# genometools/vstree

Hardware: AMD Instinct MI355X
Metric: queries/sec (100 bp queries, vmatch -mum -l 20 semantics, 3 Gbp ESA index resident in HBM) (higher is better)
Workload: dtype u8; 1 GPU; 3 Gbp synthetic DNA index, 10 M x 100 bp queries per GPU, -mum -l 20; index_bp=3000000000, queries_per_gpu=10000000, query_len=100, minlen=20, prefixlength=13, index_bytes_hbm=115012207262, reads_in_hbm=two bits per symbol, 32 bytes per read (vsa_pack_reads), parallelism=index replicated, queries sharded x1

## Files before the change

vstree_amd/csrc/api.hip:

```cpp
#include "vsa_internal.hpp"
#include <atomic>
#include <thread>
#include <time.h>
#include <algorithm>

static thread_local char g_errbuf[VSA_ERRBUF_SIZE] = "";

extern "C" char *vsa_errbuf()
{
  return g_errbuf;
}

extern "C" const char *vsa_messagespace(void)
{
  return g_errbuf;
}

int vsa_set_device(int device)
{
  VSA_HIP(hipSetDevice(device));
  return 0;
}

extern "C" int vsa_device_count(void)
// ... 382 lines not shown
  int rc = vsa_index_alloc(src->n, src->pl, src->numofchars, src->nllv,
                           src->bwt != nullptr, device, &ix, false);
  auto fail = [&](int code) {
    vsa_index_close(ix);
    return code;
  };
  if (rc != 0)
  {
    return fail(rc);
  }
  if (ix->isize != src->isize)
  {
    (void) hipFree(ix->suf);
    (void) hipFree(ix->llv);
    (void) hipFree(ix->bck);
    ix->suf = ix->llv = ix->bck = nullptr;
    ix->isize = src->isize;
    if (vsa_hip_malloc(&ix->suf, (src->n + 1) * ix->isize) != hipSuccess ||
        vsa_hip_malloc(&ix->llv, 2 * src->nllv * ix->isize + 16) != hipSuccess ||
        vsa_hip_malloc(&ix->bck, 2 * ix->numofcodes * ix->isize) != hipSuccess)
    {
      VSA_ERROR("vsa_index_clone: out of device memory");
      return fail(-100);
    }
  }
  const uint64_t n = src->n;
  struct Piece
  {
    void **dst;
    const void *from;
    uint64_t bytes;
    bool allocate;
  };
  const uint64_t ncodes = src->D > 0 ? 1ull << (2 * src->D) : 0,
                 nblocks = (n >> 6) + 1, nwaves = (nblocks + 63) / 64;
  Piece pieces[] = {
      {(void **) &ix->tis_alloc, src->tis_alloc,
       VSA_TIS_FRONTPAD + n + VSA_TIS_BACKPAD, false},
      {&ix->suf, src->suf, (n + 1) * src->isize, false},
      {(void **) &ix->lcp, src->lcp, n + 1 + 32, false},
      {&ix->llv, src->llv, 2 * src->nllv * src->isize, false},
      {&ix->bck, src->bck, 2 * src->numofcodes * src->isize, false},
      {(void **) &ix->bwt, src->bwt, n + 1 + 32, false},
      {(void **) &ix->esa8, src->esa8, (n + 1) * 8 + 64, true},
      {(void **) &ix->bck2, src->bck2, 2 * ncodes * 4 + 16, true},
      {(void **) &ix->slot16, src->slot16,
       (uint64_t) src->slotwords * ncodes * 8 + 32, true},
      {(void **) &ix->tis2, src->tis2, nblocks * 16 + 64, true},
      {(void **) &ix->spec64, src->spec64, nwaves * 8 + 64, true}};
  for (const Piece &p : pieces)
  {
    if (p.from == nullptr || p.bytes == 0)
    {
      continue;
    }
    if (p.allocate)
    {
      if (vsa_hip_malloc(p.dst, p.bytes) != hipSuccess)
      {
        VSA_ERROR("vsa_index_clone: out of device memory");
        return fail(-100);
      }
      ix->device_bytes += p.bytes;
    }
    const hipError_t e =
        hipMemcpyPeerAsync(*p.dst, device, p.from, src->device, p.bytes,
                           ix->stream);
    if (e != hipSuccess)
    {
      VSA_ERROR("vsa_index_clone: copy from device %d to device %d: %s",
                src->device, device, hipGetErrorString(e));
      return fail(-100);
    }
  }
  if (hipStreamSynchronize(ix->stream) != hipSuccess)
  {
    VSA_ERROR("vsa_index_clone: copy failed");
    return fail(-100);
  }
  ix->device_bytes = src->device_bytes;
  ix->D = src->D;
  ix->tune = src->tune;
  ix->walkshift = src->walkshift;
  ix->qspeedup = src->qspeedup;
  ix->slotwords = src->slotwords;
  ix->firstspecial = src->firstspecial;
  ix->querysepposition = src->querysepposition;
  ix->hasindexedqueries = src->hasindexedqueries;
  ix->lcpquirk = src->lcpquirk;
  *clone = ix;
  return 0;
}

extern "C" void vsa_index_close(vsa_index *ix)
{
  if (ix == nullptr)
  {
    return;
  }
  (void) hipSetDevice(ix->device);
  (void) hipFree(ix->tis_alloc);
  (void) hipFree(ix->suf);
  (void) hipFree(ix->lcp);
  (void) hipFree(ix->llv);
  (void) hipFree(ix->bck);
  (void) hipFree(ix->bwt);
  (void) hipFree(ix->esa8);
  (void) hipFree(ix->bck2);
  (void) hipFree(ix->slot16);
  (void) hipFree(ix->tis2);
  (void) hipFree(ix->spec64);
  (void) hipFree(ix->isa32);
  (void) hipFree(ix->repbits);
  if (ix->stream != nullptr)
  {
    vsa_dev_forget_stream(ix->stream);
    (void) hipStreamDestroy(ix->stream);
  }
  delete ix;
}

extern "C" int vsa_index_from_tables(const vsa_tables *t, int device,
                                     vsa_index **index)
{
  if (t == nullptr || index == nullptr)
  {
    VSA_ERROR("vsa_index_from_tables: NULL argument");
    return -1;
  }
  *index = nullptr;
  if (t->integersize != 32 && t->integersize != 64)
  {
    VSA_ERROR("integersize=%u: only 32 and 64 bit indexes are supported",
              t->integersize);
    return -2;
  }
  if ((t->tis == nullptr && t->bck != nullptr) || t->suf == nullptr ||
      t->lcp == nullptr || (t->largelcpvalues > 0 && t->llv == nullptr))
  {
    VSA_ERROR("tables tis, suf, lcp (and llv) are required");
    return -3;
  }
  if (t->numofchars == 0 || t->numofchars > 253 ||
      (t->bck != nullptr && t->prefixlength == 0))
  {
    VSA_ERROR("prefixlength=%u numofchars=%u: not a usable bucket table",
              t->prefixlength, t->numofchars);
    return -4;
  }
  vsa_index *ix = nullptr;
  int rc = vsa_index_alloc(t->totallength,
                           t->bck != nullptr ? t->prefixlength : 0,
                           t->numofchars, t->largelcpvalues,
                           t->bwt != nullptr, device, &ix);
  if (rc != 0)
  {
    vsa_index_close(ix);
    return rc;
  }
  ix->querysepposition = t->querysepposition;
  ix->hasindexedqueries = t->hasindexedqueries;
  const uint64_t n = ix->n;
  hipStream_t s = ix->stream;
  auto fail = [&](int code) {
    vsa_index_close(ix);
    return code;
// ... 980 lines not shown
```

vstree_amd/csrc/esa_search.hip:

```cpp
#include "search_host.hpp"
#include <rocprim/rocprim.hpp>
#include <type_traits>

#include "search_complete.inc"
#include "search_query.inc"
#include "mum_workplan.inc"
#include "mem_workplan.inc"
#include "mum_filter.inc"
#include "candidate_sort.inc"
#include <atomic>


namespace
{


enum class Form
{
  Ref,
  Deep,
  Staged,
  Rows,
  Windows
};
// ... 660 lines not shown
  VSA_HIP(plan_summary(st));
  st.fromplan = true;
  st.plansearches = nq;
  return 0;
}

int dump_planfile(QueryRun &st, const char *pf)
{
  const uint64_t k = std::min<uint64_t>(st.queries->nq, 65536);
  std::vector<uint32_t> hc(k), hp(k * VSA_PLAN_RANGES);
  VSA_HIP(hipMemcpyAsync(hc.data(), st.wcount.p, k * 4,
                         hipMemcpyDeviceToHost, st.stream));
  VSA_HIP(hipMemcpyAsync(hp.data(), st.wplan.p, k * sizeof(PlanRanges),
                         hipMemcpyDeviceToHost, st.stream));
  VSA_HIP(hipStreamSynchronize(st.stream));
  if (FILE *f = fopen(pf, "wb"))
  {
    for (uint64_t q = 0; q < k; q++)
    {
      (void) fwrite(&hc[q], 4, 1, f);
      (void) fwrite(&hp[q * VSA_PLAN_RANGES], 4, VSA_PLAN_RANGES, f);
    }
    fclose(f);
  }
  return 0;
}

template <typename IDX>
int mum_plan(QueryRun &st, const DevIndex<IDX> &ix)
{
  const uint64_t nq = st.queries->nq;
  if (alloc_first(st) || st.wlist.alloc(nq * 4))
  {
    return -100;
  }
  VSA_HIP(hipMemsetAsync(st.wcount.as<uint32_t>() + nq, 0, 4, st.stream));
  const uint64_t nb = blocksfor(nq), nbr = vsa_grid_blocks(nb);
  DevBuf bcount;
  if (bcount.alloc((nbr + 1) * 8) || st.wboffset.alloc((nbr + 1) * 8))
  {
    return -100;
  }
  VSA_HIP(hipMemsetAsync(bcount.as<uint64_t>() + nb, 0, 8, st.stream));
  if (first_pass(st, ix, st.form, bcount.as<uint64_t>()))
  {
    return -100;
  }
  VSA_HIP(rocprim_run(st.wtemp, [&](void *p, size_t &tb) {
    return rocprim::exclusive_scan(p, tb, bcount.as<uint64_t>(),
                                   st.wboffset.as<uint64_t>(), (uint64_t) 0,
                                   (size_t) (nb + 1), rocprim::plus<uint64_t>(),
                                   st.stream);
  }));
  k_wanted_fill<<<vsa_grid(nb), VSA_BLOCK, 0, st.stream>>>(
      st.wcount.as<uint32_t>(), nq, 0u, st.wboffset.as<uint64_t>(),
      st.wlist.as<uint32_t>());
  VSA_HIP(hipGetLastError());
  st.nlistword = st.wboffset.as<uint64_t>() + nb;
  PlanEmit em = PlanEmit();
  if (st.form != Form::Ref && plan_emit(st, VSA_PLAN_ROUNDS - 1, &em))
  {
    return -100;
  }
  withform(st.form, [&](auto deep, auto, auto rows, auto) {
    k_mum_plan<IDX, deep, deep, rows><<<gridfor(nq), VSA_BLOCK, 0, st.stream>>>(
        ix, st.qs, st.wlist.as<uint32_t>(), st.nlistword, st.searchlength,
        st.wfirste.as<uint32_t>(), st.wcount.as<uint32_t>(),
        st.wplan.as<PlanRanges>(), em);
  });
  if (st.planemit)
  {
    VSA_HIP(plan_summary(st));
  }
  VSA_HIP(hipGetLastError());
  const char *pf = getenv("VSA_DEBUG_PLANFILE");
  if (pf != nullptr && dump_planfile(st, pf))
  {
    return -100;
  }
  st.fromplan = true;
  return 0;
}

template <typename IDX>
void launch_search(QueryRun &st, const DevIndex<IDX> &ix,
                   uint64_t nplanblocks)
{
  withform(st.form, [&](auto deep, auto, auto rows, auto) {
    auto planned = [&](auto mum) {
      k_query_search_planned<IDX, 256, deep, rows, mum>
          <<<vsa_grid(nplanblocks), 256, 0, st.stream>>>(
              ix, st.qs, st.dbase, st.perquery, st.wplan.as<PlanRanges>(),
              st.wcount.as<uint32_t>(), st.searchlength,
              st.rawout.as<vsa_match>(), st.rawkeys.as<uint64_t>(),
              st.shardcap, VSA_CURSOR_SHARDS - 1,
              st.cursor.as<unsigned long long>(), st.rec.packbits,
              st.rec.valbits, st.blocksum.as<PlannedWork>(),
              st.index->walkshift);
    };
    auto unplanned = [&](auto mum) {
      k_query_search<IDX, mum, deep, 256>
          <<<vsa_grid((st.nitems + 255) / 256), 256, 0, st.stream>>>(
              ix, st.qs, st.dbase, st.perquery, st.nitems, st.searchlength,
              st.rawout.as<vsa_match>(), st.rawkeys.as<uint64_t>(),
              st.shardcap, VSA_CURSOR_SHARDS - 1,
              st.cursor.as<unsigned long long>(), st.rec.packbits,
              st.rec.valbits);
    };
    if (st.fromplan && st.domum)
    {
      planned(std::true_type());
    } else if (st.fromplan)
    {
      if constexpr (deep && !rows)
      {
        planned(std::false_type());
      }
    } else if (st.nitems > 0 && st.domum)
    {
      unplanned(std::true_type());
    } else if (st.nitems > 0)
    {
      unplanned(std::false_type());
    }
  });
}

template <typename IDX>
int search(QueryRun &st, const DevIndex<IDX> &ix)
{
  const uint32_t nshards = VSA_CURSOR_SHARDS;
  const uint64_t perblock = 256 * (st.domum ? VSA_WALK_READS : 1);
  const uint64_t nplanblocks = (st.queries->nq + perblock - 1) / perblock;
  size_t rbytes = 0;
  if (st.fromplan)
  {
    if (st.blocksum.alloc((vsa_grid_blocks(nplanblocks) + 1) *
                          sizeof(PlannedWork)))
    {
      return -100;
    }
    VSA_HIP(rocprim::reduce(nullptr, rbytes, st.blocksum.as<PlannedWork>(),
                            (PlannedWork *) nullptr, PlannedWork{0, 0},
                            (size_t) nplanblocks, PlannedWorkPlus(),
                            st.stream));
    if (st.rtemp.alloc(rbytes))
    {
      return -100;
    }
  }
  if (st.cursor.alloc((size_t) nshards * VSA_CURSOR_STRIDE * 8) ||
      st.doff.alloc(nshards * 8) || st.summary.alloc(6 * 8))
  {
    return -100;
  }
  st.shardcap =
      std::max<uint64_t>((st.queries->nq * 2 / nshards) * 5 / 4 + 64, 256);
  uint64_t maxshard = 0;
  for (int attempt = 0; attempt < 2; attempt++)
  {
    if (st.rawout.alloc(nshards * st.shardcap * st.rec.recsize) ||
        st.rawkeys.alloc(nshards * st.shardcap * 8))
    {
      return -100;
    }
    VSA_HIP(hipMemsetAsync(st.cursor.p, 0,
                           (size_t) nshards * VSA_CURSOR_STRIDE * 8,
                           st.stream));
    st.tsearch.start();
    launch_search(st, ix, nplanblocks);
    st.tsearch.stop();
    VSA_HIP(hipGetLastError());
    if (st.fromplan)
    {
      VSA_HIP(rocprim::reduce(
          st.rtemp.p, rbytes, st.blocksum.as<PlannedWork>(),
          reinterpret_cast<PlannedWork *>(st.summary.as<uint64_t>() + 4),
          PlannedWork{0, 0}, (size_t) nplanblocks, PlannedWorkPlus(),
          st.stream));
    }
    const uint64_t *sm = st.summary.as<uint64_t>();
    VSA_HIP(shard_summary(st.cursor.as<unsigned long long>(), nshards,
                          st.doff.as<uint64_t>(), st.summary.as<uint64_t>(),
                          st.stream));
    const Fetch f[8] = {{sm, 8}, {sm + 1, 8}, {sm + 2, 8}, {sm + 3, 8},
                        {sm + 4, 8}, {st.planemit ? st.psummary.p : sm, 8},
                        {st.nlistword != nullptr ? st.nlistword : sm, 8},
                        {sm + 5, 8}};
    uint64_t got[8];
    if (fetchwords(st.stream, f, 8, got))
    {
      return -100;
    }
    if (st.nlistword != nullptr)
    {
      st.nfirst = got[6] >> 32;
      st.plansearches = 2 * (got[6] & 0xFFFFFFFFull);
    }
    st.nplan = st.planemit ? got[5] : 0;
    st.needed = got[0];
    maxshard = got[1];
    st.plannedlocates = st.fromplan ? got[4] : 0;
    st.plannedwork = st.fromplan ? got[7] : 0;
    st.searchms += st.tsearch.ms();
    if (maxshard <= st.shardcap)
    {
      return 0;
    }
    st.shardcap = maxshard;
  }
  VSA_ERROR("match buffer overflow: %llu > %llu",
            (unsigned long long) maxshard, (unsigned long long) st.shardcap);
  return -5;
}

int compact(QueryRun &st)
{
  const uint64_t total = st.needed + st.nplan + st.nfirst;
  if (total == 0)
  {
    return 0;
  }
  if (st.out.alloc(total * st.rec.recsize) || st.keys.alloc(total * 8) ||
      (st.nplan > 0 &&
       compact_into(st.rec, st.prawout, st.prawkeys, st.pcap, st.pcursor,
                    st.pdoff, st.out, st.keys, st.needed, st.stream)) ||
      (st.needed > 0 &&
       compact_into(st.rec, st.rawout, st.rawkeys, st.shardcap, st.cursor,
                    st.doff, st.out, st.keys, 0, st.stream)))
  {
    return -100;
  }
  if (st.nfirst > 0)
  {
    k_append_first<<<gridfor(st.queries->nq), VSA_BLOCK, 0, st.stream>>>(
        st.wfmlen.as<uint32_t>(), st.wfmdb.as<uint64_t>(),
        st.wboffset.as<uint64_t>(), st.queries->nq, st.perquery, st.dbase,
        st.qs.seqoffset, st.needed + st.nplan, st.out.as<vsa_match>(),
        st.keys.as<uint64_t>(), st.rec.packbits, st.rec.valbits);
    VSA_HIP(hipGetLastError());
  }
  st.needed = total;
  return 0;
}

#define VSA_CS_MINPAIRS (1u << 14)

std::atomic<uint64_t> g_cs_runs{0}, g_cs_overflows{0}, g_cs_longruns{0},
    g_cs_shift{0}, g_cs_buckets{0};

bool feedsbuckets(const QueryRun &st)
{
  const uint64_t total = st.needed + st.nplan + st.nfirst;
  const uint32_t tune = st.index->tune;
  if (!(st.domum && !st.domumcand && st.rec.packed && (tune & 4u) == 0 &&
        total > 0 && (total >= VSA_CS_MINPAIRS || (tune & 8u) != 0) &&
        cs_geometry(st.index->n, total, st.rec.lenbits, st.rec.dbbits)
                .nbuckets <= VSA_CS_MAXBUCKETS))
  {
    return false;
  }
  if ((tune & 8u) == 0 && st.index->cs_skip > 0)
  {
    st.index->cs_skip--;
    return false;
  }
  return true;
}

template <typename VAL>
int mumfilter_buckets(QueryRun &st, DevBuf &mums, MumCounts *c)
{
  const RecordForm &rec = st.rec;
  const uint64_t total = st.needed + st.nplan + st.nfirst;
  CsSources src = CsSources();
  if (st.needed > 0)
  {
    src.reg[0] = {st.rawout.p, st.rawkeys.as<uint64_t>(),
                  st.cursor.as<unsigned long long>(), st.shardcap, st.needed};
  }
  if (st.nplan > 0)
  {
    src.reg[1] = {st.prawout.p, st.prawkeys.as<uint64_t>(),
                  st.pcursor.as<unsigned long long>(), st.pcap, st.nplan};
  }
  if (st.nfirst > 0)
  {
    src.first = {st.wfmlen.as<uint32_t>(), st.wfmdb.as<uint64_t>(),
                 st.queries->nq, st.qs.seqoffset, rec.packbits, rec.valbits};
  }
  CsGeometry g;
  if (mums.alloc(total * sizeof(vsa_match)))
// ... 548 lines not shown
```

vstree_amd/csrc/index_derive.hip:

```cpp
#include "search_host.hpp"
#include <rocprim/rocprim.hpp>


template <typename IDX>
__global__ void __launch_bounds__(VSA_BLOCK)
k_make_esa8(const uint8_t *__restrict__ tis, const IDX *__restrict__ suf,
            const uint8_t *__restrict__ lcp, uint64_t count, uint32_t D,
            uint64_t *__restrict__ esa8)
{
  const uint64_t j = vsa_bid() * VSA_BLOCK + threadIdx.x;
  if (j >= count)
  {
    return;
  }
  const uint64_t s = suf[j];
  const uint8_t *t = tis + s + D;
  uint64_t key = 0, flag = 0;
#pragma unroll
  for (uint32_t k = 0; k < VSA_KEYSYMS; k++)
  {
    const uint8_t a = t[k];
    if (VSA_ISSPECIAL(a))
    {
      flag = VSA_KEYFLAG;
// ... 21 lines not shown
#pragma unroll
    for (int k = 0; k < 4; k++)
    {
      const vsa_u128 v = vsa_load16(p + 16 * k);
      const uint64_t notdna = 0xFCFCFCFCFCFCFCFCull;
      const uint64_t s0 = v.lo & notdna, s1 = v.hi & notdna;
      if (firstbad == ~0ull && (s0 | s1) != 0)
      {
        firstbad = 64 * b + 16 * k +
                   (s0 != 0 ? ((uint64_t) __builtin_ctzll(s0) >> 3)
                            : 8 + ((uint64_t) __builtin_ctzll(s1) >> 3));
      }
      const uint64_t packed = vsa_pack16(v.lo, v.hi);
      out[k >> 1] |= packed << (32 * (1 - (k & 1)));
    }
    out[0] = __builtin_bswap64(out[0]);
    out[1] = __builtin_bswap64(out[1]);
    reinterpret_cast<uint64_t *>(tis2)[2 * b] = out[0];
    reinterpret_cast<uint64_t *>(tis2)[2 * b + 1] = out[1];
    special = firstbad != ~0ull || 64 * b + 64 > n;
    if (firstbad != ~0ull)
    {
      atomicMin(firstspecial, (unsigned long long) firstbad);
    }
  }
  const uint64_t mask = __ballot(special);
  if ((threadIdx.x & 63) == 0 && b < nblocks)
  {
    reinterpret_cast<uint64_t *>(spec64)[b >> 6] = mask;
  }
}

template <int W, typename IDX>
__global__ void __launch_bounds__(VSA_BLOCK)
k_make_slots(const IDX *__restrict__ bck2, const uint64_t *__restrict__ esa8,
             uint64_t ncodes, uint64_t *__restrict__ slot,
             unsigned int *__restrict__ toobig)
{
  for (uint64_t c = vsa_bid() * VSA_BLOCK + threadIdx.x;
       c < ncodes; c += vsa_nblocks() * VSA_BLOCK)
  {
    const IDX left = bck2[2 * c], mid = bck2[2 * c + 1];
    if constexpr (sizeof(IDX) == 4)
    {
      slot[W * c] = (uint64_t) left | ((uint64_t) mid << 32);
    } else
    {
      const uint64_t cnt = mid > left ? mid - left : 0;
      if (cnt >> (64 - VSA_WIDE_LEFTBITS) != 0)
      {
        *toobig = 1;
      }
      slot[W * c] = left | (cnt << VSA_WIDE_LEFTBITS);
    }
#pragma unroll
    for (int k = 0; k + 1 < W; k++)
    {
      slot[W * c + 1 + k] = (mid > left + k) ? esa8[left + k] : 0;
    }
  }
}

int vsa_index_make_esa8(vsa_index *ix)
{
  const char *off = getenv("VSA_NO_ESA8");
  {
    const char *tn = getenv("VSA_TUNE"), *wc = getenv("VSA_WALK_CHUNK");
    const int asked = wc != nullptr ? atoi(wc) : 0;
    ix->tune = tn != nullptr ? (uint32_t) atoi(tn) : 0;
    uint32_t chunk = VSA_WALK_CHUNK;
    if (asked >= 1 && asked <= 0x8000)
    {
      chunk = (uint32_t) asked;
    }
    if ((ix->tune & 16u) != 0)
    {
      chunk = 1;
    }
    ix->walkshift = 0;
    while ((2u << ix->walkshift) <= chunk)
    {
      ix->walkshift++;
    }
  }
  if (ix->esa8 != nullptr)
  {
    (void) hipFree(ix->esa8);
    ix->esa8 = nullptr;
  }
  if (ix->bck2 != nullptr)
  {
    (void) hipFree(ix->bck2);
    ix->bck2 = nullptr;
  }
  if (ix->slot16 != nullptr)
  {
    (void) hipFree(ix->slot16);
    ix->slot16 = nullptr;
  }
  if (ix->tis2 != nullptr)
  {
    (void) hipFree(ix->tis2);
    (void) hipFree(ix->spec64);
    ix->tis2 = ix->spec64 = nullptr;
  }
  const bool wide = ix->isize != 4;
  if (ix->numofchars != 4 || ix->bck == nullptr ||
      (wide && ((ix->n + 1) >> VSA_WIDE_LEFTBITS) != 0) ||
      (off != nullptr && strcmp(off, "1") == 0))
  {
    return 0;
  }
  uint32_t D = 1;
  while (D < 16 && (1ull << (2 * D)) < ix->n)
  {
    D++;
  }
  if (D < ix->pl)
  {
    D = ix->pl;
  }
  const char *fd = getenv("VSA_DEEP_PREFIX");
  if (fd != nullptr && atoi(fd) >= (int) ix->pl && atoi(fd) <= 16)
  {
    D = (uint32_t) atoi(fd);
  } else
  {
    size_t freeb = 0, totalb = 0;
    const uint32_t wanted = D;
    (void) hipStreamSynchronize(ix->stream);
    vsa_dev_trim();
    while (D > ix->pl && D > 12 &&
           hipMemGetInfo(&freeb, &totalb) == hipSuccess)
    {
      const uint64_t codes = 1ull << (2 * D),
                     need = 16 * codes + 2 * codes * ix->isize +
                            8 * (ix->n + 1) + ix->n / 4 + totalb / 10;
      if (need <= freeb)
      {
        break;
      }
      D--;
    }
    const char *tr = getenv("VSA_TRACE");
    if (tr != nullptr && strcmp(tr, "0") != 0)
    {
      fprintf(stderr, "vstree_amd: derived tables: deep prefix %u (wanted %u; "
              "%.1f GB free of %.1f on the device)\n", D, wanted,
              (double) freeb / 1e9, (double) totalb / 1e9);
    }
  }
  if (D > 16)
  {
    return 0;
  }
  static_assert(VSA_TIS_BACKPAD >= 16 + VSA_KEYSYMS + 8, "text pad too small");
  ix->D = D;
  const uint64_t count = ix->n + 1, ncodes = 1ull << (2 * D);
  VSA_HIP(hipStreamSynchronize(ix->stream));
  vsa_dev_trim();
  if (vsa_hip_malloc((void **) &ix->slot16, 2 * ncodes * 8 + 32) != hipSuccess)
  {
    (void) hipGetLastError();
    ix->slot16 = nullptr;
    ix->D = 0;
    return 0;
// ... 96 lines not shown
```

vstree_amd/csrc/mum_walk.inc:

```
template <typename IDX, bool DEEP, bool PQ, typename QP>
__device__ __forceinline__ uint32_t
vsa_walk_chunk(const DevIndex<IDX> &ix, const DevQueries &qs, bool active,
               QP read, const RowQuery *rq, uint32_t qlen, uint32_t first,
               uint32_t off, uint64_t q, const uint64_t *__restrict__ base,
               uint32_t perquery, uint32_t searchlength,
               vsa_match *__restrict__ out, uint64_t *__restrict__ outkey,
               uint64_t shardcap, uint32_t shard,
               unsigned long long *__restrict__ cursors, uint32_t packbits,
               uint32_t valbits)
{
  uint32_t locates = 0;
  while (__any(active))
  {
    uint32_t c = 0, maxlcp = 0;
    uint64_t witness = 0;
    uint8_t leftchar = (uint8_t) VSA_SEPARATOR;
    const uint32_t remaining = qlen - off;
    const QP qptr = read + off;
    bool have = false, fast = false;
    DeepHit hit;
    int st = VSA_LOC_SLOW;
    locates += active ? 1u : 0u;
    if (active && off > 0)
    {
      if constexpr (PQ)
      {
        leftchar = (uint8_t) (vsa_pq_window(*rq, off - 1) >> 62);
      } else
      {
        leftchar = vsa_qsym(read, off - 1);
      }
    }
    if constexpr (DEEP)
    {
      const uint32_t qleft = off > 0 ? (uint32_t) leftchar : 0x100u;
      if constexpr (PQ)
      {
        st = vsa_locate_deep<1, true>(ix, active, qptr, remaining, maxlcp,
                                      witness, hit, searchlength, qleft, rq,
                                      off);
      } else
      {
        st = vsa_locate_deep(ix, active, qptr, remaining, maxlcp, witness,
                             hit, searchlength, qleft);
      }
    }
    if (st == VSA_LOC_SLOW)
    {
      have = active &&
             vsa_locate_reference(ix, qptr, remaining, maxlcp, witness);
    } else
    {
      have = st == VSA_LOC_FOUND;
      fast = have && maxlcp < 255;
    }
    const bool cutshort = st != VSA_LOC_SLOW && hit.notleftmax;
    if (have && maxlcp >= searchlength && !cutshort)
    {
      if (fast)
      {
        const uint32_t lcpw = (uint32_t) (hit.ew >> 32) & 0xFFu;
        const bool unique = (witness == 0 || lcpw < maxlcp) &&
                            (witness + 1 > ix.n - 1 || hit.lcpnext < maxlcp);
        c = (unique && (VSA_ISSPECIAL(leftchar) || leftchar != hit.leftsym))
                ? 1u
                : 0u;
      } else
      {
        c = (vsa_mum_candidate<IDX, DEEP>(ix, maxlcp, witness) &&
             vsa_leftmaximal(ix, vsa_sufstart<IDX, DEEP>(ix, witness),
                             leftchar))
                ? 1u
                : 0u;
      }
    }
    const uint64_t inshard = vsa_wave_reserve01(
        cursors + (uint64_t) shard * VSA_CURSOR_STRIDE, c != 0);
    if (c != 0 && inshard < shardcap)
    {
      const uint64_t dbstart = fast ? vsa_entrystart(ix, hit.ew, witness)
                                    : vsa_sufstart<IDX, DEEP>(ix, witness);
      const uint64_t t0 = (base != nullptr) ? base[q] : q * perquery;
      vsa_write_candidate(qs, out, outkey,
                          (uint64_t) shard * shardcap + inshard, q, off,
                          t0 + off, dbstart, maxlcp, packbits, valbits);
    }
    if (active)
    {
      uint32_t bound;
      if (st == VSA_LOC_SLOW)
      {
        bound = have ? maxlcp : ix.pl - 1;
      } else
      {
        bound = have ? maxlcp : ix.D - 1;
      }
      const uint32_t reach = off + bound;
      uint32_t next = off - 1;
      bool left = off > first;
      if (!cutshort && reach + 1 < off + searchlength)
      {
        left = left && reach >= searchlength;
        next = reach - searchlength;
      }
      active = left && next >= first;
      off = next;
    }
  }
  return locates;
}
```

vstree_amd/csrc/mum_workplan.inc:

```



#define VSA_PLAN_RANGES 4
#define VSA_PLAN_ROUNDS 6
#define VSA_PLAN_UNKNOWN 0xFFFFFFFFu

#ifndef VSA_PLAN_WAVES
#define VSA_PLAN_WAVES 1
#endif
#ifndef VSA_FIRST_WAVES
#define VSA_FIRST_WAVES 1
#endif
struct PlanRanges
{
  uint32_t r[VSA_PLAN_RANGES];
};

__device__ __forceinline__ void plan_add(PlanRanges &pr, uint32_t &nr,
                                         uint32_t first, uint32_t last)
{
  if (first > last)
  {
    return;
  }
// ... 457 lines not shown
      }
      q = q0 + lo;
      if constexpr (!MUM)
      {
        t0 = (base != nullptr) ? base[q] : q * perquery;
      }
      if constexpr (MUM && !ROWS)
      {
        if (qs.dense)
        {
          qstart = qs.symbols + q * qs.uniformlen;
        } else
        {
          qstart = qs.symbols + qs.start[q];
          qlen = (uint32_t) qs.length[q];
        }
      }
    }
    if constexpr (!MUM)
    {
      vsa_query_item<IDX, false, DEEP>(ix, qs, active, q, off, t0 + off,
                                       searchlength, out, outkey, shardcap,
                                       shard, cursors, 0, 0);
      continue;
    }
    if constexpr (DEEP && ROWS)
    {
      RowQuery rq;
      QSrc src;
      bool flagged = false;
      rq.row = qs.rows;
      rq.valid = 0;
      src.row = qs.rows;
      src.bytes = nullptr;
      src.pos = src.m = 0;
      if (active)
      {
        flagged = vsa_row_of(qs, q, qs.uniformlen, rq, src);
      }
      locates += vsa_walk_chunk<IDX, true, true>(
          ix, qs, active && !flagged, src, &rq, qlen, first, off, q, base,
          perquery, searchlength, out, outkey, shardcap, shard, cursors,
          packbits, valbits);
      if (__any(active && flagged))
      {
        locates += vsa_walk_chunk<IDX, true, false>(
            ix, qs, active && flagged, src, nullptr, qlen, first, off, q, base,
            perquery, searchlength, out, outkey, shardcap, shard, cursors,
            packbits, valbits);
      }
    } else
    {
      locates += vsa_walk_chunk<IDX, DEEP, false>(
          ix, qs, active, qstart, nullptr, qlen, first, off, q, base, perquery,
          searchlength, out, outkey, shardcap, shard, cursors, packbits,
          valbits);
    }
  }
  if constexpr (MUM)
  {
#pragma unroll
    for (int d = 32; d >= 1; d >>= 1)
    {
      locates += __shfl_xor(locates, d, 64);
    }
    if ((tid & 63u) == 0)
    {
      wavelocates[tid >> 6] = locates;
    }
    __syncthreads();
    if (tid == 0)
    {
      uint32_t s = 0;
#pragma unroll
      for (int w = 0; w < BLK / 64; w++)
      {
        s += wavelocates[w];
      }
      blocksum[vsa_bid()].locates = s;
    }
  }
}

template <typename IDX, bool DEEP, bool PQ = false, bool ROWS = false,
          bool WINDOWS = false>
__global__ void __launch_bounds__(VSA_BLOCK, VSA_FIRST_WAVES)
k_mum_first(const DevIndex<IDX> ix, const DevQueries qs, uint32_t perquery,
            uint32_t searchlength, uint32_t *__restrict__ count,
            uint32_t *__restrict__ firste, uint32_t *__restrict__ fmlen,
            uint64_t *__restrict__ fmdb,
            uint64_t *__restrict__ blockcount = nullptr)
{
  extern __shared__ uint32_t stagedqueries[];
  __shared__ uint32_t wantwaves[VSA_BLOCK / 64], candwaves[VSA_BLOCK / 64];
  const uint64_t q = vsa_bid() * VSA_BLOCK + threadIdx.x;
  uint32_t qlen = qs.uniformlen, perq = perquery;
  const uint8_t *qptr = qs.symbols;
  uint32_t maxlcp = 0;
  uint64_t witness = 0;
  bool have = false, fast = false;
  DeepHit hit;

  if (!ROWS && q < qs.nq)
  {
    if (qs.dense)
    {
      qptr = qs.symbols + q * qs.uniformlen;
    } else
    {
      qptr = qs.symbols + qs.start[q];
      qlen = (uint32_t) qs.length[q];
      perq = (qlen >= searchlength) ? qlen - searchlength + 1 : 0;
    }
  }
  const bool active = q < qs.nq && perq > 0;
  if constexpr (DEEP && ROWS && WINDOWS)
  {
    RowQuery rq;
    QSrc src;
    bool flagged = false;
    rq.row = qs.rows;
    rq.valid = 0;
    src.row = qs.rows;
    src.bytes = nullptr;
    src.pos = src.m = 0;
    if (q < qs.nq)
    {
      flagged = vsa_row_of(qs, q, qlen, rq, src);
    }
    int st = vsa_locate_deep<3, true>(ix, active && !flagged, src, qlen,
                                      maxlcp, witness, hit, 0xFFFFFFFFu,
                                      0x100u, &rq, 0);
    if (active && flagged)
    {
      st = VSA_LOC_SLOW;
    }
    if (st == VSA_LOC_SLOW)
    {
      have = vsa_locate_reference(ix, src, qlen, maxlcp, witness);
    } else
    {
      have = st == VSA_LOC_FOUND;
      fast = have && maxlcp < 255;
    }
  } else if constexpr (DEEP && ROWS)
  {
    PackedQuery pq;
    QSrc src;
    pq.w[0] = pq.w[1] = pq.w[2] = pq.w[3] = 0;
    pq.valid = 0;
    src.row = qs.rows;
    src.bytes = nullptr;
    src.pos = src.m = 0;
    if (q < qs.nq)
    {
      vsa_pq_from_row(qs, q, qlen, pq, src);
    }
    const int st = vsa_locate_deep<3, true>(ix, active, src, qlen, maxlcp,
                                            witness, hit, 0xFFFFFFFFu, 0x100u,
                                            &pq);
    if (st == VSA_LOC_SLOW)
    {
      have = vsa_locate_reference(ix, src, qlen, maxlcp, witness);
    } else
    {
      have = st == VSA_LOC_FOUND;
// ... 182 lines not shown
```

vstree_amd/csrc/vsa_internal.hpp:

```cpp
#pragma once

#include <hip/hip_runtime.h>
#include <cstdint>
#include <cstdio>
#include <cstdlib>
#include <cstring>
#include <vector>
#include "vstree_amd.h"

extern "C" char *vsa_errbuf();
#define VSA_ERRBUF_SIZE 1024
#define VSA_ERROR(...)                                                        \
  do                                                                          \
  {                                                                           \
    snprintf(vsa_errbuf(), VSA_ERRBUF_SIZE, __VA_ARGS__);                     \
  } while (0)

#define VSA_HIP(call)                                                         \
  do                                                                          \
  {                                                                           \
    hipError_t e_ = (call);                                                   \
    if (e_ != hipSuccess)                                                     \
    {                                                                         \
      VSA_ERROR("%s:%d: %s failed: %s", __FILE__, __LINE__, #call,            \
                hipGetErrorString(e_));                                       \
      return -100;                                                            \
    }                                                                         \
  } while (0)

#define VSA_TIS_FRONTPAD 64
#define VSA_TIS_BACKPAD 64
#define VSA_QUERY_BACKPAD 64

template <typename IDX>
struct DevIndex
{
  const uint8_t *tis;
  const IDX *suf;
  const uint8_t *lcp;
  const IDX *llv;
  const IDX *bck;
  const uint8_t *bwt;
  const uint64_t *esa8;
  const uint32_t *bck2;
  const uint64_t *slot16;
  uint32_t slotwords;
  const uint8_t *tis2;
  const uint8_t *spec64;
  uint64_t firstspecial;
  uint64_t n, nllv, numofcodes;
  uint32_t pl, numofchars, D;
  uint32_t tune;
  uint32_t qspeedup;
};

#define VSA_KEYSYMS 10u
#define VSA_KEYSHIFT 40u
#define VSA_KEYMASK 0xFFFFFu
#define VSA_LEFTSHIFT 60u
#define VSA_KEYFLAG (1ull << 62)
#define VSA_LEFTSPECIAL (1ull << 63)

#ifndef VSA_WALK_CHUNK
#define VSA_WALK_CHUNK 32
#endif

struct vsa_index
{
  int device;
  hipStream_t stream;
  uint32_t isize;
  uint64_t n, nllv, numofcodes;
  uint32_t pl, numofchars;
  uint8_t *tis_alloc;
  void *suf, *llv, *bck;
  uint8_t *lcp, *bwt;
  uint64_t *esa8;
  uint32_t *bck2;
  uint64_t *slot16;
  uint32_t slotwords;
  uint8_t *tis2, *spec64;
  uint64_t firstspecial;
  uint32_t D, tune;
  uint32_t walkshift;
  uint32_t qspeedup;
  uint64_t querysepposition;
  int hasindexedqueries;
  uint64_t device_bytes;
  mutable int lcpquirk;
  mutable uint32_t *isa32;
  mutable uint32_t *repbits = nullptr;
  mutable uint32_t repleast = 0;
  mutable uint32_t cs_skip = 0, cs_penalty = 0;

  template <typename IDX>
  DevIndex<IDX> view() const
  {
    DevIndex<IDX> v;
    v.tis = tis_alloc + VSA_TIS_FRONTPAD;
    v.suf = (const IDX *) suf;
    v.lcp = lcp;
    v.llv = (const IDX *) llv;
    v.bck = (const IDX *) bck;
    v.bwt = bwt;
    v.esa8 = esa8;
    v.bck2 = bck2;
    v.slot16 = slot16;
    v.slotwords = slotwords;
    v.tis2 = tis2;
    v.spec64 = spec64;
    v.firstspecial = firstspecial;
    v.D = D;
    v.tune = tune;
    v.qspeedup = qspeedup;
    v.n = n;
    v.nllv = nllv;
    v.numofcodes = numofcodes;
    v.pl = pl;
    v.numofchars = numofchars;
    return v;
  }
};

struct vsa_queries
{
  int device;
  uint64_t nq, nsymbols;
  uint64_t *rows = nullptr;
  uint32_t roww = 0;
  uint8_t *side = nullptr;
  uint64_t nside = 0;
  bool ownsrows = true;
  mutable bool bytesvalid = false;
  uint64_t bytescapacity = 0;
  mutable uint8_t *symbols;
  uint64_t *start;
  uint64_t *length;
  uint64_t minlength, maxlength;
  uint64_t seqoffset;
  std::vector<uint64_t> hlength;
  bool uniform;
  bool dense;
  uint64_t *dnalength = nullptr;
  double translate_ms = 0.0;
};

struct vsa_result
{
  int device;
  uint64_t count;
  vsa_match *matches;
  vsa_stats stats;
  uint32_t packbits;
  uint64_t *packvals;
};

int vsa_unpack_result(const vsa_result *r, uint64_t count, vsa_match *device);

struct DevQueries
{
  const uint64_t *rows;
  const uint8_t *side;
  uint64_t nside;
  uint32_t roww;
  const uint8_t *symbols;
  const uint64_t *start;
  const uint64_t *length;
// ... 79 lines not shown
```

Measured before the change: 3.762 billion queries/s.

## Add persistent tile-queue walk kernel with dynamic per-wave chunk refill

Replaces the static planned MUM walk launch with a persistent kernel sized to the occupancy-derived grid. Each wave atomically grabs tiles of 64 queries from a global counter and refills idle lanes from a chunk queue held in LDS. This is meant to cut lane divergence and tail imbalance across the variable-length walks. The walk chunk size also drops from 32 to 8 so work is split more finely, at the cost of more atomics, LDS traffic and a fallback path with a single output region when the buffer overflows.

```diff
diff --git a/vstree_amd/csrc/api.hip b/vstree_amd/csrc/api.hip
--- a/vstree_amd/csrc/api.hip
+++ b/vstree_amd/csrc/api.hip
@@ -488,6 +488,7 @@
   ix->D = src->D;
   ix->tune = src->tune;
   ix->walkshift = src->walkshift;
+  ix->walkgridasked = src->walkgridasked;
   ix->qspeedup = src->qspeedup;
   ix->slotwords = src->slotwords;
   ix->firstspecial = src->firstspecial;
diff --git a/vstree_amd/csrc/esa_search.hip b/vstree_amd/csrc/esa_search.hip
--- a/vstree_amd/csrc/esa_search.hip
+++ b/vstree_amd/csrc/esa_search.hip
@@ -766,11 +766,61 @@
   return 0;
 }
 
+bool tilequeue(const QueryRun &st)
+{
+  return st.fromplan && st.domum && (st.index->tune & 32u) == 0;
+}
+
+template <typename IDX>
+int walkgrid(const QueryRun &st, uint32_t *grid)
+{
+  const vsa_index *index = st.index;
+  if (index->walkgridasked != 0)
+  {
+    *grid = index->walkgridasked;
+    return 0;
+  }
+  hipError_t e = hipSuccess;
+  withform(st.form, [&](auto deep, auto, auto rows, auto) {
+    uint32_t &kept = index->walkgrid[deep ? 1 : 0][rows ? 1 : 0];
+    if (kept == 0)
+    {
+      int percu = 0, cus = 0;
+      e = hipOccupancyMaxActiveBlocksPerMultiprocessor(
+          &percu, k_mum_walk_tiles<IDX, deep, rows>, 256, 0);
+      if (e == hipSuccess)
+      {
+        e = hipDeviceGetAttribute(&cus, hipDeviceAttributeMultiprocessorCount,
+                                  index->device);
+      }
+      if (e == hipSuccess)
+      {
+        kept = (uint32_t) std::max(percu, 1) * (uint32_t) std::max(cus, 1);
+      }
+    }
+    *grid = kept;
+  });
+  VSA_HIP(e);
+  return 0;
+}
+
 template <typename IDX>
 void launch_search(QueryRun &st, const DevIndex<IDX> &ix,
-                   uint64_t nplanblocks)
+                   uint64_t nplanblocks, uint32_t regions)
 {
   withform(st.form, [&](auto deep, auto, auto rows, auto) {
+    auto tiles = [&]() {
+      unsigned long long *cursors = st.cursor.as<unsigned long long>();
+      k_mum_walk_tiles<IDX, deep, rows>
+          <<<vsa_grid(nplanblocks), 256, 0, st.stream>>>(
+              ix, st.qs, st.dbase, st.perquery, st.wplan.as<PlanRanges>(),
+              st.wcount.as<uint32_t>(), st.wlist.as<uint32_t>(), st.nlistword,
+              cursors + (size_t) VSA_CURSOR_SHARDS * VSA_CURSOR_STRIDE,
+              st.searchlength, st.rawout.as<vsa_match>(),
+              st.rawkeys.as<uint64_t>(), st.shardcap, regions - 1, cursors,
+              st.rec.packbits, st.rec.valbits,
+              st.blocksum.as<PlannedWork>(), st.index->walkshift);
+    };
     auto planned = [&](auto mum) {
       k_query_search_planned<IDX, 256, deep, rows, mum>
           <<<vsa_grid(nplanblocks), 256, 0, st.stream>>>(
@@ -791,7 +841,10 @@
               st.cursor.as<unsigned long long>(), st.rec.packbits,
               st.rec.valbits);
     };
-    if (st.fromplan && st.domum)
+    if (tilequeue(st))
+    {
+      tiles();
+    } else if (st.fromplan && st.domum)
     {
       planned(std::true_type());
     } else if (st.fromplan)
@@ -815,44 +868,55 @@
 {
   const uint32_t nshards = VSA_CURSOR_SHARDS;
   const uint64_t perblock = 256 * (st.domum ? VSA_WALK_READS : 1);
-  const uint64_t nplanblocks = (st.queries->nq + perblock - 1) / perblock;
+  uint64_t nplanblocks = (st.queries->nq + perblock - 1) / perblock;
+  uint64_t persum = 1;
   size_t rbytes = 0;
+  if (tilequeue(st))
+  {
+    uint32_t grid = 0;
+    if (walkgrid<IDX>(st, &grid))
+    {
+      return -100;
+    }
+    nplanblocks = grid;
+    persum = 4;
+  }
+  const uint64_t nsums = persum * nplanblocks;
   if (st.fromplan)
   {
-    if (st.blocksum.alloc((vsa_grid_blocks(nplanblocks) + 1) *
+    if (st.blocksum.alloc((persum * vsa_grid_blocks(nplanblocks) + 1) *
                           sizeof(PlannedWork)))
     {
       return -100;
     }
     VSA_HIP(rocprim::reduce(nullptr, rbytes, st.blocksum.as<PlannedWork>(),
                             (PlannedWork *) nullptr, PlannedWork{0, 0},
-                            (size_t) nplanblocks, PlannedWorkPlus(),
-                            st.stream));
+                            (size_t) nsums, PlannedWorkPlus(), st.stream));
     if (st.rtemp.alloc(rbytes))
     {
       return -100;
     }
   }
-  if (st.cursor.alloc((size_t) nshards * VSA_CURSOR_STRIDE * 8) ||
-      st.doff.alloc(nshards * 8) || st.summary.alloc(6 * 8))
+  const size_t cursorbytes = (size_t) (nshards + 1) * VSA_CURSOR_STRIDE * 8;
+  if (st.cursor.alloc(cursorbytes) || st.doff.alloc(nshards * 8) ||
+      st.summary.alloc(6 * 8))
   {
     return -100;
   }
   st.shardcap =
       std::max<uint64_t>((st.queries->nq * 2 / nshards) * 5 / 4 + 64, 256);
   uint64_t maxshard = 0;
+  uint32_t regions = nshards;
   for (int attempt = 0; attempt < 2; attempt++)
   {
-    if (st.rawout.alloc(nshards * st.shardcap * st.rec.recsize) ||
-        st.rawkeys.alloc(nshards * st.shardcap * 8))
+    if (st.rawout.alloc(regions * st.shardcap * st.rec.recsize) ||
+        st.rawkeys.alloc(regions * st.shardcap * 8))
     {
       return -100;
     }
-    VSA_HIP(hipMemsetAsync(st.cursor.p, 0,
-                           (size_t) nshards * VSA_CURSOR_STRIDE * 8,
-                           st.stream));
+    VSA_HIP(hipMemsetAsync(st.cursor.p, 0, cursorbytes, st.stream));
     st.tsearch.start();
-    launch_search(st, ix, nplanblocks);
+    launch_search(st, ix, nplanblocks, regions);
     st.tsearch.stop();
     VSA_HIP(hipGetLastError());
     if (st.fromplan)
@@ -860,8 +924,7 @@
       VSA_HIP(rocprim::reduce(
           st.rtemp.p, rbytes, st.blocksum.as<PlannedWork>(),
           reinterpret_cast<PlannedWork *>(st.summary.as<uint64_t>() + 4),
-          PlannedWork{0, 0}, (size_t) nplanblocks, PlannedWorkPlus(),
-          st.stream));
+          PlannedWork{0, 0}, (size_t) nsums, PlannedWorkPlus(), st.stream));
     }
     const uint64_t *sm = st.summary.as<uint64_t>();
     VSA_HIP(shard_summary(st.cursor.as<unsigned long long>(), nshards,
@@ -892,6 +955,11 @@
       return 0;
     }
     st.shardcap = maxshard;
+    if (tilequeue(st))
+    {
+      regions = 1;
+      st.shardcap = st.needed;
+    }
   }
   VSA_ERROR("match buffer overflow: %llu > %llu",
             (unsigned long long) maxshard, (unsigned long long) st.shardcap);
diff --git a/vstree_amd/csrc/index_derive.hip b/vstree_amd/csrc/index_derive.hip
--- a/vstree_amd/csrc/index_derive.hip
+++ b/vstree_amd/csrc/index_derive.hip
@@ -127,6 +127,10 @@
     {
       ix->walkshift++;
     }
+    const char *wg = getenv("VSA_WALK_GRID");
+    const int grid = wg != nullptr ? atoi(wg) : 0;
+    ix->walkgridasked = (grid >= 1 && grid <= (1 << 20)) ? (uint32_t) grid : 0;
+    memset(ix->walkgrid, 0, sizeof ix->walkgrid);
   }
   if (ix->esa8 != nullptr)
   {
diff --git a/vstree_amd/csrc/mum_walk.inc b/vstree_amd/csrc/mum_walk.inc
--- a/vstree_amd/csrc/mum_walk.inc
+++ b/vstree_amd/csrc/mum_walk.inc
@@ -1,3 +1,110 @@
+template <typename IDX, bool DEEP, bool PQ, typename QP>
+__device__ __forceinline__ void
+vsa_walk_step(const DevIndex<IDX> &ix, const DevQueries &qs, bool &active,
+              QP read, const RowQuery *rq, uint32_t qlen, uint32_t first,
+              uint32_t &off, uint64_t q, const uint64_t *__restrict__ base,
+              uint32_t perquery, uint32_t searchlength,
+              vsa_match *__restrict__ out, uint64_t *__restrict__ outkey,
+              uint64_t shardcap, uint32_t shard,
+              unsigned long long *__restrict__ cursors, uint32_t packbits,
+              uint32_t valbits, uint32_t &locates)
+{
+  uint32_t c = 0, maxlcp = 0;
+  uint64_t witness = 0;
+  uint8_t leftchar = (uint8_t) VSA_SEPARATOR;
+  const uint32_t remaining = qlen - off;
+  const QP qptr = read + off;
+  bool have = false, fast = false;
+  DeepHit hit;
+  int st = VSA_LOC_SLOW;
+  locates += active ? 1u : 0u;
+  if (active && off > 0)
+  {
+    if constexpr (PQ)
+    {
+      leftchar = (uint8_t) (vsa_pq_window(*rq, off - 1) >> 62);
+    } else
+    {
+      leftchar = vsa_qsym(read, off - 1);
+    }
+  }
+  if constexpr (DEEP)
+  {
+    const uint32_t qleft = off > 0 ? (uint32_t) leftchar : 0x100u;
+    if constexpr (PQ)
+    {
+      st = vsa_locate_deep<1, true>(ix, active, qptr, remaining, maxlcp,
+                                    witness, hit, searchlength, qleft, rq,
+                                    off);
+    } else
+    {
+      st = vsa_locate_deep(ix, active, qptr, remaining, maxlcp, witness,
+                           hit, searchlength, qleft);
+    }
+  }
+  if (st == VSA_LOC_SLOW)
+  {
+    have = active &&
+           vsa_locate_reference(ix, qptr, remaining, maxlcp, witness);
+  } else
+  {
+    have = st == VSA_LOC_FOUND;
+    fast = have && maxlcp < 255;
+  }
+  const bool cutshort = st != VSA_LOC_SLOW && hit.notleftmax;
+  if (have && maxlcp >= searchlength && !cutshort)
+  {
+    if (fast)
+    {
+      const uint32_t lcpw = (uint32_t) (hit.ew >> 32) & 0xFFu;
+      const bool unique = (witness == 0 || lcpw < maxlcp) &&
+                          (witness + 1 > ix.n - 1 || hit.lcpnext < maxlcp);
+      c = (unique && (VSA_ISSPECIAL(leftchar) || leftchar != hit.leftsym))
+              ? 1u
+              : 0u;
+    } else
+    {
+      c = (vsa_mum_candidate<IDX, DEEP>(ix, maxlcp, witness) &&
+           vsa_leftmaximal(ix, vsa_sufstart<IDX, DEEP>(ix, witness),
+                           leftchar))
+              ? 1u
+              : 0u;
+    }
+  }
+  const uint64_t inshard = vsa_wave_reserve01(
+      cursors + (uint64_t) shard * VSA_CURSOR_STRIDE, c != 0);
+  if (c != 0 && inshard < shardcap)
+  {
+    const uint64_t dbstart = fast ? vsa_entrystart(ix, hit.ew, witness)
+                                  : vsa_sufstart<IDX, DEEP>(ix, witness);
+    const uint64_t t0 = (base != nullptr) ? base[q] : q * perquery;
+    vsa_write_candidate(qs, out, outkey,
+                        (uint64_t) shard * shardcap + inshard, q, off,
+                        t0 + off, dbstart, maxlcp, packbits, valbits);
+  }
+  if (active)
+  {
+    uint32_t bound;
+    if (st == VSA_LOC_SLOW)
+    {
+      bound = have ? maxlcp : ix.pl - 1;
+    } else
+    {
+      bound = have ? maxlcp : ix.D - 1;
+    }
+    const uint32_t reach = off + bound;
+    uint32_t next = off - 1;
+    bool left = off > first;
+    if (!cutshort && reach + 1 < off + searchlength)
+    {
+      left = left && reach >= searchlength;
+      next = reach - searchlength;
+    }
+    active = left && next >= first;
+    off = next;
+  }
+}
+
 template <typename IDX, bool DEEP, bool PQ, typename QP>
 __device__ __forceinline__ uint32_t
 vsa_walk_chunk(const DevIndex<IDX> &ix, const DevQueries &qs, bool active,
@@ -12,100 +119,10 @@
   uint32_t locates = 0;
   while (__any(active))
   {
-    uint32_t c = 0, maxlcp = 0;
-    uint64_t witness = 0;
-    uint8_t leftchar = (uint8_t) VSA_SEPARATOR;
-    const uint32_t remaining = qlen - off;
-    const QP qptr = read + off;
-    bool have = false, fast = false;
-    DeepHit hit;
-    int st = VSA_LOC_SLOW;
-    locates += active ? 1u : 0u;
-    if (active && off > 0)
-    {
-      if constexpr (PQ)
-      {
-        leftchar = (uint8_t) (vsa_pq_window(*rq, off - 1) >> 62);
-      } else
-      {
-        leftchar = vsa_qsym(read, off - 1);
-      }
-    }
-    if constexpr (DEEP)
-    {
-      const uint32_t qleft = off > 0 ? (uint32_t) leftchar : 0x100u;
-      if constexpr (PQ)
-      {
-        st = vsa_locate_deep<1, true>(ix, active, qptr, remaining, maxlcp,
-                                      witness, hit, searchlength, qleft, rq,
-                                      off);
-      } else
-      {
-        st = vsa_locate_deep(ix, active, qptr, remaining, maxlcp, witness,
-                             hit, searchlength, qleft);
-      }
-    }
-    if (st == VSA_LOC_SLOW)
-    {
-      have = active &&
-             vsa_locate_reference(ix, qptr, remaining, maxlcp, witness);
-    } else
-    {
-      have = st == VSA_LOC_FOUND;
-      fast = have && maxlcp < 255;
-    }
-    const bool cutshort = st != VSA_LOC_SLOW && hit.notleftmax;
-    if (have && maxlcp >= searchlength && !cutshort)
-    {
-      if (fast)
-      {
-        const uint32_t lcpw = (uint32_t) (hit.ew >> 32) & 0xFFu;
-        const bool unique = (witness == 0 || lcpw < maxlcp) &&
-                            (witness + 1 > ix.n - 1 || hit.lcpnext < maxlcp);
-        c = (unique && (VSA_ISSPECIAL(leftchar) || leftchar != hit.leftsym))
-                ? 1u
-                : 0u;
-      } else
-      {
-        c = (vsa_mum_candidate<IDX, DEEP>(ix, maxlcp, witness) &&
-             vsa_leftmaximal(ix, vsa_sufstart<IDX, DEEP>(ix, witness),
-                             leftchar))
-                ? 1u
-                : 0u;
-      }
-    }
-    const uint64_t inshard = vsa_wave_reserve01(
-        cursors + (uint64_t) shard * VSA_CURSOR_STRIDE, c != 0);
-    if (c != 0 && inshard < shardcap)
-    {
-      const uint64_t dbstart = fast ? vsa_entrystart(ix, hit.ew, witness)
-                                    : vsa_sufstart<IDX, DEEP>(ix, witness);
-      const uint64_t t0 = (base != nullptr) ? base[q] : q * perquery;
-      vsa_write_candidate(qs, out, outkey,
-                          (uint64_t) shard * shardcap + inshard, q, off,
-                          t0 + off, dbstart, maxlcp, packbits, valbits);
-    }
-    if (active)
-    {
-      uint32_t bound;
-      if (st == VSA_LOC_SLOW)
-      {
-        bound = have ? maxlcp : ix.pl - 1;
-      } else
-      {
-        bound = have ? maxlcp : ix.D - 1;
-      }
-      const uint32_t reach = off + bound;
-      uint32_t next = off - 1;
-      bool left = off > first;
-      if (!cutshort && reach + 1 < off + searchlength)
-      {
-        left = left && reach >= searchlength;
-        next = reach - searchlength;
-      }
-      active = left && next >= first;
-      off = next;
-    }
+    vsa_walk_step<IDX, DEEP, PQ>(ix, qs, active, read, rq, qlen, first, off, q,
+                                 base, perquery, searchlength, out, outkey,
+                                 shardcap, shard, cursors, packbits, valbits,
+                                 locates);
   }
   return locates;
 }
diff --git a/vstree_amd/csrc/mum_workplan.inc b/vstree_amd/csrc/mum_workplan.inc
--- a/vstree_amd/csrc/mum_workplan.inc
+++ b/vstree_amd/csrc/mum_workplan.inc
@@ -563,6 +563,269 @@
   }
 }
 
+struct WalkTile
+{
+  PlanRanges pr[64];
+  uint32_t q[64];
+  uint32_t pre[65];
+};
+#define VSA_WALK_ASIDE 128
+struct WalkAside
+{
+  uint32_t q[VSA_WALK_ASIDE], r[VSA_WALK_ASIDE];
+};
+
+__device__ __forceinline__ void vsa_wave_lds_fence()
+{
+  __builtin_amdgcn_fence(__ATOMIC_RELEASE, "wavefront");
+  __builtin_amdgcn_wave_barrier();
+  __builtin_amdgcn_fence(__ATOMIC_ACQUIRE, "wavefront");
+}
+
+__device__ __forceinline__ uint32_t vsa_rank_in(uint64_t mask)
+{
+  return __builtin_amdgcn_mbcnt_hi(
+      (uint32_t) (mask >> 32), __builtin_amdgcn_mbcnt_lo((uint32_t) mask, 0u));
+}
+
+__device__ __forceinline__ void vsa_plan_chunk(const PlanRanges &p, uint32_t r,
+                                               uint32_t cshift,
+                                               uint32_t &first, uint32_t &off)
+{
+  const uint32_t chunk = 1u << cshift;
+#pragma unroll
+  for (int k = 0; k < VSA_PLAN_RANGES; k++)
+  {
+    const uint32_t rf = p.r[k] & 0xFFFFu, len = p.r[k] >> 16,
+                   nchunks = (len + chunk - 1) >> cshift;
+    if (r < nchunks)
+    {
+      const uint32_t at = r << cshift, n = len - at < chunk ? len - at : chunk;
+      first = rf + at;
+      off = first + n - 1;
+      r = 0xFFFFFFFFu;
+    } else if (r != 0xFFFFFFFFu)
+    {
+      r -= nchunks;
+    }
+  }
+}
+
+template <typename IDX, bool DEEP = true, bool ROWS = false>
+__global__ void __launch_bounds__(256, VSA_WALK_WAVES)
+k_mum_walk_tiles(const DevIndex<IDX> ix, const DevQueries qs,
+                 const uint64_t *__restrict__ base, uint32_t perquery,
+                 const PlanRanges *__restrict__ plan,
+                 const uint32_t *__restrict__ plancount,
+                 const uint32_t *__restrict__ list,
+                 const uint64_t *__restrict__ nlistword,
+                 unsigned long long *__restrict__ tilecounter,
+                 uint32_t searchlength, vsa_match *__restrict__ out,
+                 uint64_t *__restrict__ outkey, uint64_t shardcap,
+                 uint32_t shardmask, unsigned long long *__restrict__ cursors,
+                 uint32_t packbits, uint32_t valbits,
+                 PlannedWork *__restrict__ blocksum, uint32_t chunkshift)
+{
+  __shared__ WalkTile tiles[4];
+  __shared__ WalkAside asides[ROWS ? 4 : 1];
+  const uint32_t lane = threadIdx.x & 63u, wave = threadIdx.x >> 6;
+  WalkTile &tile = tiles[wave];
+  WalkAside &aside = asides[ROWS ? wave : 0];
+  const uint64_t nlist = *nlistword & 0xFFFFFFFFull;
+  const uint32_t shard = vsa_bid() & shardmask;
+  uint32_t head = 0, tail = 0, naside = 0;
+  bool exhausted = false;
+  bool active = false;
+  uint32_t off = 0, first = 0, q = 0, qlen = qs.uniformlen;
+  uint32_t locates = 0, offsets = 0;
+  const uint8_t *qstart = qs.symbols;
+  for (;;)
+  {
+    uint64_t freemask = __ballot(!active);
+    while (freemask != 0 && !(ROWS && naside >= 64))
+    {
+      if (head == tail)
+      {
+        if (exhausted)
+        {
+          break;
+        }
+        unsigned long long mine = 0;
+        if (lane == 0)
+        {
+          mine = atomicAdd(tilecounter, 1ull);
+        }
+        const uint64_t t0 =
+            ((uint64_t) __builtin_amdgcn_readfirstlane((uint32_t) (mine >> 32))
+             << 32) |
+            __builtin_amdgcn_readfirstlane((uint32_t) mine);
+        if (t0 * 64 >= nlist)
+        {
+          exhausted = true;
+          break;
+        }
+        const uint64_t t = t0 * 64 + lane;
+        uint32_t tq = 0, nch = 0;
+        PlanRanges p;
+#pragma unroll
+        for (int g = 0; g < VSA_PLAN_RANGES; g++)
+        {
+          p.r[g] = 0;
+        }
+        if (t < nlist)
+        {
+          tq = list[t];
+          const uint32_t c = plancount[tq];
+          p = plan[tq];
+          offsets += c;
+          if (c > 0)
+          {
+#pragma unroll
+            for (int g = 0; g < VSA_PLAN_RANGES; g++)
+            {
+              nch += ((p.r[g] >> 16) + (1u << chunkshift) - 1) >> chunkshift;
+            }
+          }
+        }
+        const uint32_t incl = vsa_wave_inclusive_sum(nch);
+        vsa_wave_lds_fence();
+        tile.q[lane] = tq;
+        tile.pr[lane] = p;
+        tile.pre[lane + 1] = incl;
+        if (lane == 0)
+        {
+          tile.pre[0] = 0;
+        }
+        vsa_wave_lds_fence();
+        head = 0;
+        tail = __builtin_amdgcn_readlane(incl, 63);
+        continue;
+      }
+      const uint32_t nfree = (uint32_t) __popcll(freemask),
+                     take = nfree < tail - head ? nfree : tail - head,
+                     rank = vsa_rank_in(freemask);
+      const bool took = !active && rank < take;
+      bool flagged = false;
+      if (took)
+      {
+        const uint32_t i = head + rank;
+        uint32_t lo = 0;
+#pragma unroll
+        for (uint32_t d = 32; d >= 1; d >>= 1)
+        {
+          if (tile.pre[lo + d] <= i)
+          {
+            lo += d;
+          }
+        }
+        q = tile.q[lo];
+        vsa_plan_chunk(tile.pr[lo], i - tile.pre[lo], chunkshift, first, off);
+        if constexpr (ROWS)
+        {
+          RowQuery rq;
+          QSrc src;
+          flagged = vsa_row_of(qs, q, qs.uniformlen, rq, src);
+        } else
+        {
+          if (qs.dense)
+          {
+            qstart = qs.symbols + (uint64_t) q * qs.uniformlen;
+          } else
+          {
+            qstart = qs.symbols + qs.start[q];
+            qlen = (uint32_t) qs.length[q];
+          }
+        }
+        active = !flagged;
+      }
+      head += take;
+      if constexpr (ROWS)
+      {
+        const uint64_t fmask = __ballot(flagged);
+        if (flagged)
+        {
+          const uint32_t at = naside + vsa_rank_in(fmask);
+          aside.q[at] = q;
+          aside.r[at] = first | (off << 16);
+        }
+        naside += (uint32_t) __popcll(fmask);
+      }
+      freemask = __ballot(!active);
+    }
+    if (!__any(active))
+    {
+      if constexpr (ROWS)
+      {
+        if (naside > 0)
+        {
+          vsa_wave_lds_fence();
+          for (uint32_t a0 = 0; a0 < naside; a0 += 64)
+          {
+            const bool mine = a0 + lane < naside;
+            uint32_t aq = 0, afirst = 0, aoff = 0;
+            RowQuery arq;
+            QSrc src;
+            arq.row = qs.rows;
+            arq.valid = 0;
+            src.row = qs.rows;
+            src.bytes = nullptr;
+            src.pos = src.m = 0;
+            if (mine)
+            {
+              aq = aside.q[a0 + lane];
+              afirst = aside.r[a0 + lane] & 0xFFFFu;
+              aoff = aside.r[a0 + lane] >> 16;
+              (void) vsa_row_of(qs, aq, qs.uniformlen, arq, src);
+            }
+            locates += vsa_walk_chunk<IDX, true, false>(
+                ix, qs, mine, src, nullptr, qlen, afirst, aoff, aq, base,
+                perquery, searchlength, out, outkey, shardcap, shard, cursors,
+                packbits, valbits);
+          }
+          vsa_wave_lds_fence();
+          naside = 0;
+          q = first = off = 0;
+          continue;
+        }
+      }
+      break;
+    }
+    if constexpr (DEEP && ROWS)
+    {
+      RowQuery rq;
+      QSrc src;
+      rq.row = qs.rows + (uint64_t) q * qs.roww;
+      rq.valid = qlen;
+      src.row = rq.row;
+      src.bytes = nullptr;
+      src.pos = 0;
+      src.m = (int32_t) qlen;
+      vsa_walk_step<IDX, true, true>(ix, qs, active, src, &rq, qlen, first,
+                                     off, q, base, perquery, searchlength, out,
+                                     outkey, shardcap, shard, cursors, packbits,
+                                     valbits, locates);
+    } else
+    {
+      vsa_walk_step<IDX, DEEP, false>(ix, qs, active, qstart, nullptr, qlen,
+                                      first, off, q, base, perquery,
+                                      searchlength, out, outkey, shardcap,
+                                      shard, cursors, packbits, valbits,
+                                      locates);
+    }
+  }
+  uint64_t sum = locates | ((uint64_t) offsets << 32);
+#pragma unroll
+  for (int d = 32; d >= 1; d >>= 1)
+  {
+    sum += vsa_shfl64(sum, (int) lane ^ d);
+  }
+  if (lane == 0)
+  {
+    blocksum[vsa_bid() * 4 + wave] =
+        PlannedWork{sum & 0xFFFFFFFFull, sum >> 32};
+  }
+}
+
 template <typename IDX, bool DEEP, bool PQ = false, bool ROWS = false,
           bool WINDOWS = false>
 __global__ void __launch_bounds__(VSA_BLOCK, VSA_FIRST_WAVES)
diff --git a/vstree_amd/csrc/vsa_internal.hpp b/vstree_amd/csrc/vsa_internal.hpp
--- a/vstree_amd/csrc/vsa_internal.hpp
+++ b/vstree_amd/csrc/vsa_internal.hpp
@@ -62,7 +62,7 @@
 #define VSA_LEFTSPECIAL (1ull << 63)
 
 #ifndef VSA_WALK_CHUNK
-#define VSA_WALK_CHUNK 32
+#define VSA_WALK_CHUNK 8
 #endif
 
 struct vsa_index
@@ -83,6 +83,8 @@
   uint64_t firstspecial;
   uint32_t D, tune;
   uint32_t walkshift;
+  uint32_t walkgridasked;
+  mutable uint32_t walkgrid[2][2];
   uint32_t qspeedup;
   uint64_t querysepposition;
   int hasindexedqueries;
```

Result: faster. 4.104 billion queries/s, median of 6 (+9.1%).
